# lynet55/robotic-mpc

Hardware: AMD Instinct MI355X
Metric: MPC-steps/sec (whole node), UR10 N=100 dt=0.01 batch; 1/2/4/8 GPU (higher is better)
Workload: dtype f64

## Files before the change

### robotic_mpc_amd/csrc/mpc_core.h

```cpp
#pragma once
#include "mpc_kin.h"
#include "mpc_ipm.h"
#include "mpc_nlp.h"

#define MPC_REP16(X) X(0) X(1) X(2) X(3) X(4) X(5) X(6) X(7) X(8) X(9) X(10) X(11) X(12) X(13) X(14) X(15)
#define MPC_REP4(X) X(0) X(1) X(2) X(3)

namespace mpcb {

constexpr double BOUND_INF = 1e29;

constexpr int L1 = 98;
constexpr int L2N = 62;
constexpr int L2W = 114;

#ifndef MPCB_FUSE
#define MPCB_FUSE 1
#endif
#ifdef MPCB_PROFILE
#define PROF_T0(v) const double v = ex.clock()
#define PROF_ADD(i, v) prof[i] += ex.clock() - v
#else
#define PROF_T0(v)
#define PROF_ADD(i, v)
// ... 590 lines not shown
                            }
                        }
                    });
                }
                ex.par([&](int lane) {
                    ex.put_max(sm.red[0], lane, a_s.at(lane)); ex.put_max(sm.red[1], lane, a_e.at(lane));
                    ex.put_max(sm.red[2], lane, a_i.at(lane)); ex.put_max(sm.red[3], lane, a_c.at(lane));
                });
                rs = fmax(rs, ex.get_max(sm.red[0]));
                re = fmax(re, ex.get_max(sm.red[1]));
                ri = fmax(ri, ex.get_max(sm.red[2]));
                rc = fmax(rc, ex.get_max(sm.red[3]));
            }
            copies([&](int lane, auto nl) {
                constexpr int NL = decltype(nl)::value;
                if (wide) copy_lanes<W2, 0, W2, L2W, false, NL>(v2, ex.smem().w.G2, k0, k1, lane);
                else copy_lanes<W2_LIN, 0, W2, L2N, false, NL>(v2, ex.smem().w.G2, k0, k1, lane);
            });
            PROF_ADD(PF_X3, tn);
        }
        if (res4) { res4[0] = rs; res4[1] = re; res4[2] = ri; res4[3] = rc; }
        PROF_ADD(PF_NLP, t0);
        return cost;
    }

    MPC_PASS void residual_direct(int mode, double a)
    {
        PROF_T0(t0);
        Smem &sm = ex.smem();
        const InstParams &P = sm.P;
        const int Nl = ex.uni(ex.smem().n_hor), NS = Nl + 1;
        double *const G1 = ex.smem().w.G1, *const G2 = ex.smem().w.G2, *const G3 = ex.smem().w.G3;
        double *const Y = ex.pool();
        a = ex.uni(a);
        typename Ex::template PerLane<double> n_g, n_b, n_d, n_m, n_mu, n_c;
        PROF_T0(tx);
        ex.wpar([&](int lane) { n_g.at(lane) = 0; n_b.at(lane) = 0; n_d.at(lane) = 0; n_m.at(lane) = 0; n_mu.at(lane) = 0; n_c.at(lane) = 0; });
        if (mode == 1) {
            constexpr int IPS = 15, R = rounds_for(IPS);
            const int items = NS * IPS;
            for (int base = 0; base < items; base += R * NT) {
                ex.wpar([&](int lane) {
                    D2 cur[R], stp[R];
#pragma unroll
                    for (int r = 0; r < R; r++) {
                        const int e = imin(base + r * NT + lane, items - 1), k = e / IPS, c = 2 * (e - k * IPS);
                        cur[r] = *(MPC_GLOBAL const D2 *)(G1 + (size_t)k * W1 + O_QW + c);
                        stp[r] = *(MPC_GLOBAL const D2 *)(G3 + (size_t)(c >= 18 ? imin(k + 1, Nl) : k) * W3 + O_DW + c);
                    }
#pragma unroll
                    for (int r = 0; r < R; r++) {
                        const int e = base + r * NT + lane;
                        if (e < items) {
                            const int k = e / IPS, c = 2 * (e - k * IPS);
                            const double aa = (c >= 18 && k >= Nl) ? 0.0 : a;
                            D2 v = cur[r];
                            v.x += aa * stp[r].x; v.y += aa * stp[r].y;
                            *(MPC_GLOBAL D2 *)(G1 + (size_t)k * W1 + O_QW + c) = v;
                        }
                    }
                });
            }
        } else {
            ex.wpar([&](int lane) {
                if (lane < NX) gst(G1 + O_QW + 6 + lane, sm.xhat[lane] - gld(G1 + O_X + lane));
                if (lane >= 16 && lane < 16 + NU) gst(G1 + (size_t)Nl * W1 + O_QW + lane - 16, 0.0);
            });
        }
        {
            constexpr int IPS = 24, R = rounds_for(IPS);
            const int items = NS * IPS;
            for (int base = 0; base < items; base += R * NT) {
                ex.wpar([&](int lane) {
                    D2 cur[R], stp[R];
#pragma unroll
                    for (int r = 0; r < R; r++) {
                        const int e = imin(base + r * NT + lane, items - 1), k = e / IPS, q = 2 * (e - k * IPS);
                        cur[r] = *(MPC_GLOBAL const D2 *)(G1 + (size_t)k * W1 + O_QLAM + q);
                        if (mode == 1) stp[r] = *(MPC_GLOBAL const D2 *)(G3 + (size_t)k * W3 + O_DLAM + q);
                    }
                    double ncl = n_c.at(lane);
#pragma unroll
                    for (int r = 0; r < R; r++) {
                        const int e = base + r * NT + lane;
                        if (e < items) {
                            const int k = e / IPS, q = 2 * (e - k * IPS);
                            const bool is_t = q >= 24;
                            const int sc = is_t ? q - 24 : q, j = sc < 12 ? sc : sc - 12;
                            const bool ok = j < 6 ? k < Nl : (k >= 1 && k < Nl);
                            const D2 m = *reinterpret_cast<const D2 *>(&sm.bon[sc]);
                            const bool on0 = ok && m.x != 0.0, on1 = ok && m.y != 0.0;
                            D2 v = cur[r];
                            if (mode == 1) {
                                v.x = ipm::step_floor(on0, v.x, a, stp[r].x); v.y = ipm::step_floor(on1, v.y, a, stp[r].y);
                            } else {
                                v.x = is_t ? ipm::warm_t(on0, v.x) : ipm::warm_lam(on0, v.x);
                                v.y = is_t ? ipm::warm_t(on1, v.y) : ipm::warm_lam(on1, v.y);
                                ncl += (on0 && !is_t ? 1.0 : 0.0) + (on1 && !is_t ? 1.0 : 0.0);
                            }
                            *(MPC_GLOBAL D2 *)(G1 + (size_t)k * W1 + O_QLAM + q) = v;
                        }
                    }
                    n_c.at(lane) = ncl;
                });
            }
        }
        ex.barrier();
        PROF_ADD(PF_X1, tx);
        PROF_T0(ty);
        const int CY = ex.uni(imax(1, imin(ex.smem().pool_n / 6, NS)));
        for (int y0 = 0; y0 < NS; y0 += CY) {
        const int y1 = imin(y0 + CY, NS);
        if (y0 > 0) ex.barrier();
        {
            constexpr int R = rounds_for(NTASK);
            const int items = (imin(y1, Nl) - y0) * NTASK;
            for (int base = 0; base < items; base += R * NT) {
                ex.wpar([&](int lane) {
                    double g[R][12], d[R][12], rr[R];
#pragma unroll
                    for (int r = 0; r < R; r++) {
                        const int e = imax(imin(base + r * NT + lane, items - 1), 0), k = y0 + e / NTASK, i = e - (k - y0) * NTASK;
                        const double *g1 = G1 + (size_t)k * W1 + O_QW, *g2 = G2 + (size_t)k * W2;
                        rr[r] = gld(g2 + O_R + i);
#pragma unroll
                        for (int j = 0; j < 6; j++) { g[r][j] = gld(g2 + O_GQ + i * 6 + j); d[r][j] = gld(g1 + 6 + j); }
                        if (i == 4) {
#pragma unroll
                            for (int j = 0; j < 6; j++) { g[r][6 + j] = gld(g2 + O_GV + j); d[r][6 + j] = gld(g1 + 12 + j); }
                        }
                    }
#pragma unroll
                    for (int r = 0; r < R; r++) {
                        const int e = base + r * NT + lane;
                        if (e < items) {
                            const int k = y0 + e / NTASK, i = e - (k - y0) * NTASK;
                            double v = rr[r];
#pragma unroll
                            for (int j = 0; j < 6; j++) v += g[r][j] * d[r][j];
                            if (i == 4) {
#pragma unroll
                                for (int j = 0; j < 6; j++) v += g[r][6 + j] * d[r][6 + j];
                            }
                            v *= P.w_task[i];
                            Y[(k - y0) * 6 + i] = v;
                            gst(G2 + (size_t)k * W2 + O_Y + i, v);
                        }
                    }
                });
            }
        }
        ex.barrier();
        PROF_ADD(PF_X2, ty);
        PROF_T0(tz);
        {
            constexpr int R = Ex::VGPR_BUDGET <= 256 && rounds_for(6) > 2 ? 2 : rounds_for(6);
            const int items = (y1 - y0) * 6;
            const double dt = P.dt, lm = P.lm;
            auto bounds = [&](int lane, int k, int ci, double val_, double dv, double l_lo, double l_hi, double t_lo, double t_hi,
                              double &rg) {
                const bool hc = ci < 6 ? k < Nl : (k >= 1 && k < Nl);
                const bool blo = hc && sm.bon[ci] != 0.0, bhi = hc && sm.bon[12 + ci] != 0.0;
                const double val = hc ? val_ : 0.0;
                const double ll = blo ? l_lo : 0.0, lu = bhi ? l_hi : 0.0;
                const double itl = fast_rcp(t_lo), itu = fast_rcp(t_hi);
                const double rdl = blo ? dv - (bnd_lo(P, ci) - val) - t_lo : 0.0;
                const double rdu = bhi ? (bnd_hi(P, ci) - val) - dv - t_hi : 0.0;
                const double rml = ll * t_lo, rmu = lu * t_hi;
                double gt = rg;
                rg -= ll; gt -= ll;
                double gam = ll * itl;
                gt += (rml + ll * rdl) * itl;
                rg += lu; gt += lu;
                gam += lu * itu;
                gt -= (rmu + lu * rdu) * itu;
                n_mu.at(lane) += rml + rmu;
                n_d.at(lane) = fmax(n_d.at(lane), fmax(fabs(rdl), fabs(rdu)));
                n_m.at(lane) = fmax(n_m.at(lane), fmax(fabs(rml), fabs(rmu)));
                double *g3 = G3 + (size_t)k * W3, *g2 = G2 + (size_t)k * W2;
                gst(g3 + O_RD + ci, rdl); gst(g3 + O_RD + 12 + ci, rdu);
                gst(g3 + O_RM + ci, rml); gst(g3 + O_RM + 12 + ci, rmu);
                gst(g2 + O_GAM + ci, gam);
                return gt;
            };
            constexpr int RD = 2 * R;
            const int items_d = (y1 - y0) * NX;
            for (int base = 0; base < items; base += R * NT) {
                ex.wpar([&](int lane) {
                    double v[R][12], q[R][13], d[RD][5];
#pragma unroll
                    for (int r = 0; r < R; r++) {
                        const int e = imin(base + r * NT + lane, items - 1), k = y0 + e / 6, j = e - (k - y0) * 6, km = imax(k - 1, 0);
                        const double *g1 = G1 + (size_t)k * W1, *g2 = G2 + (size_t)k * W2, *gm = G1 + (size_t)km * W1;
                        v[r][0] = gld(g1 + O_U + j);      v[r][1] = gld(g1 + O_X + 6 + j);
                        v[r][2] = gld(g1 + O_QW + j);     v[r][3] = gld(g1 + O_QW + 12 + j);
                        v[r][4] = gld(g1 + O_QPI + j);    v[r][5] = gld(g1 + O_QPI + 6 + j);
                        v[r][6] = gld(gm + O_QPI + 6 + j);
                        v[r][7] = gld(g2 + O_GV + j);
                        v[r][8] = gld(g1 + O_QLAM + j);   v[r][9] = gld(g1 + O_QLAM + 12 + j);
                        v[r][10] = gld(g1 + O_QT + j);    v[r][11] = gld(g1 + O_QT + 12 + j);
                        q[r][0] = gld(g1 + O_X + j);  q[r][1] = gld(g1 + O_QW + 6 + j);
#pragma unroll
                        for (int i = 0; i < NTASK; i++) q[r][2 + i] = gld(g2 + O_GQ + i * 6 + j);
                        q[r][7] = v[r][4]; q[r][8] = gld(gm + O_QPI + j);
                        q[r][9] = gld(g1 + O_QLAM + 6 + j);  q[r][10] = gld(g1 + O_QLAM + 18 + j);
                        q[r][11] = gld(g1 + O_QT + 6 + j);   q[r][12] = gld(g1 + O_QT + 18 + j);
                    }
#pragma unroll
                    for (int r = 0; r < RD; r++) {
                        const int e = imin(2 * base + r * NT + lane, items_d - 1), k = y0 + e / NX, i = e - (k - y0) * NX, kn = imin(k + 1, Nl);
                        const double *dw = G1 + (size_t)k * W1 + O_QW;
                        d[r][0] = gld(dw + 6 + i);
                        d[r][1] = gld(dw + (i < 6 ? 12 + i : i - 6));
                        d[r][2] = gld(dw + (i < 6 ? i : i - 6));
                        d[r][3] = gld(G2 + (size_t)k * W2 + O_BD + i);
                        d[r][4] = gld(G1 + (size_t)kn * W1 + O_QW + 6 + i);
                    }
#pragma unroll
                    for (int r = 0; r < R; r++) {
                        const int e = base + r * NT + lane;
                        if (e < items) {
                            const int k = y0 + e / 6, j = e - (k - y0) * 6;
                            const double du = v[r][2], dvv = v[r][3];
                            const double uj = v[r][0] + du, vj = v[r][1] + dvv;
                            const double c2 = P.w_qddot * P.cq[j] * P.cq[j];
                            double *g3 = G3 + (size_t)k * W3, *g2 = G2 + (size_t)k * W2;
                            double rgu = 0.0;
                            if (k < Nl) {
                                rgu = dt * (2.0 * P.w_u * uj + c2 * (uj - vj));
                                rgu += P.b1[j] * v[r][4] + P.b2[j] * v[r][5];
                                rgu += dt * lm * du;
                            }
                            const double gtu = bounds(lane, k, j, v[r][0], du, v[r][8], v[r][9], v[r][10], v[r][11], rgu);
                            gst(g3 + O_RG + j, rgu); gst(g2 + O_GT + j, gtu);
                            double rgv = 0.0;
                            if (k >= 1) {
                                if (k < Nl) {
                                    rgv = dt * (v[r][7] * Y[(k - y0) * 6 + 4] + c2 * (vj - uj));
                                    rgv += P.a12[j] * v[r][4] + P.a22[j] * v[r][5];
                                }
                                rgv += (k < Nl ? dt : 1.0) * lm * dvv;
                                rgv -= v[r][6];
                            }
                            gst(g3 + O_RG + 12 + j, rgv); gst(g2 + O_GT + 12 + j, rgv);
                            const double dq = q[r][1];
                            double rg = 0.0;
                            if (k >= 1) {
                                if (k < Nl) {
                                    double s_ = 0.0;
#pragma unroll
                                    for (int i = 0; i < NTASK; i++) s_ += q[r][2 + i] * Y[(k - y0) * 6 + i];
                                    rg = dt * s_ + q[r][7];
                                }
                                rg += (k < Nl ? dt : 1.0) * lm * dq;
                                rg -= q[r][8];
                            }
                            const double gt = bounds(lane, k, 6 + j, q[r][0], dq, q[r][9], q[r][10], q[r][11], q[r][12], rg);
                            gst(g3 + O_RG + 6 + j, rg); gst(g2 + O_GT + 6 + j, gt);
                            n_g.at(lane) = fmax(n_g.at(lane), fmax(fmax(fabs(rgu), fabs(rgv)), fabs(rg)));
                        }
                    }
#pragma unroll
                    for (int r = 0; r < RD; r++) {
                        const int e = 2 * base + r * NT + lane;
                        if (e < items_d && e < 2 * (base + R * NT)) {
                            const int k = y0 + e / NX, i = e - (k - y0) * NX;
                            double vv = 0.0;
                            if (k < Nl) {
                                if (i < 6) vv = d[r][0] + P.a12[i] * d[r][1] + P.b1[i] * d[r][2];
                                else vv = P.a22[i - 6] * d[r][0] + P.b2[i - 6] * d[r][1];
                                vv += d[r][3] - d[r][4];
                                n_b.at(lane) = fmax(n_b.at(lane), fabs(vv));
                            }
                            gst(G2 + (size_t)k * W2 + O_RB + i, vv);
                        }
                    }
                });
            }
        }
        PROF_ADD(PF_X3, tz);
        }
        ex.par([&](int lane) {
            ex.put_max(sm.red[0], lane, n_g.at(lane)); ex.put_max(sm.red[1], lane, n_b.at(lane));
            ex.put_max(sm.red[2], lane, n_d.at(lane)); ex.put_max(sm.red[3], lane, n_m.at(lane));
            ex.put_sum(sm.red[4], lane, n_mu.at(lane)); ex.put_sum(sm.red[5], lane, n_c.at(lane));
        });
        const double ng = ex.get_max(sm.red[0]), nb = ex.get_max(sm.red[1]), nd = ex.get_max(sm.red[2]), nm = ex.get_max(sm.red[3]);
        const double smu = ex.get_sum(sm.red[4]), nc = ex.get_sum(sm.red[5]);
        ex.par([&](int lane) {
            if ((lane & (WAVE - 1)) == 0) {
                sm.ret[0] = ng; sm.ret[1] = nb; sm.ret[2] = nd; sm.ret[3] = nm; sm.ret[4] = smu;
                if (mode == 0) sm.ret[5] = nc;
            }
        });
        PROF_ADD(PF_RES, t0);
    }

    struct FactLane {
        double b1a, b2a, b1b, b2b, a12a, a22a, a12b, a22b;
        double hu_c;
        double huv_c;
        double lm_c;
        double mqq, mqv, mvq, mvv;
        double qqq, qqv, qvq, qvv;
        int a, b;
        int oqq, oqv, ovv;
    };

    template <int MODE>
    MPC_PASS void fact_pass_t()
    {
        constexpr bool RES = MODE == 1, SEG = MODE == 2;
        PROF_T0(t0);
        Smem &sm = ex.smem();
        const InstParams &P = sm.P;
        const int Nl = ex.uni(ex.smem().n_hor);
        constexpr int WR = 78;
        constexpr int WF = RES ? W4 - O_PM : W4;
        constexpr int FO = RES ? O_PM : 0;
        const ResMap rm = res_map();
        const int CH = RES ? chunk_len_in(rm.scr_n, 2 * (WR + WF), 2 * WR) : chunk_len(2 * (WR + W4), 2 * WR);
        typename Ex::template PerLane<FactLane> fl;
        ex.seq([&](int lane) {
            FactLane &f = fl.at(lane);
            const int a = lane < 36 ? lane / 6 : 0, b = lane < 36 ? lane % 6 : 0;
            f.a = a; f.b = b;
            f.oqq = tri(imin(a, b), imax(a, b)); f.oqv = tri(a, 6 + b); f.ovv = tri(6 + imin(a, b), 6 + imax(a, b));
            f.b1a = P.b1[a]; f.b2a = P.b2[a]; f.b1b = P.b1[b]; f.b2b = P.b2[b];
            f.a12a = P.a12[a]; f.a22a = P.a22[a]; f.a12b = P.a12[b]; f.a22b = P.a22[b];
            const double c2 = P.dt * P.w_qddot * P.cq[a] * P.cq[a];
            f.hu_c = a == b ? P.dt * 2.0 * P.w_u + c2 + P.dt * P.lm : 0.0;
            f.huv_c = a == b ? c2 : 0.0;
            f.lm_c = a == b ? P.dt * P.lm : 0.0;
            f.mqq = f.mqv = f.mvq = f.mvv = 0.0;
            f.qqq = f.qqv = f.qvq = f.qvv = 0.0;
        });
        const double dw0 = P.dt * P.w_task[0], dw1 = P.dt * P.w_task[1], dw2 = P.dt * P.w_task[2], dw3 = P.dt * P.w_task[3],
                     dw4 = P.dt * P.w_task[4];
        auto next_stage = [&](int lane, FactLane &f, double gam_u, int sb) {
            const double fq = f.b1a * f.mqq + f.b2a * f.mvq, fv = f.b1a * f.mqv + f.b2a * f.mvv;
            double r = fq * f.b1b + fv * f.b2b + f.hu_c;
            r += f.a == f.b ? gam_u : 0.0;
            sm.Rt[f.a * 6 + f.b] = r;
            double *St = sm.St2[sb];
            St[f.a * 12 + f.b] = fq;
            St[f.a * 12 + 6 + f.b] = fq * f.a12b + fv * f.a22b - f.huv_c;
            const double cq = f.a12a * f.mqq + f.a22a * f.mvq, cv = f.a12a * f.mqv + f.a22a * f.mvv;
            f.qqq = f.mqq;
            f.qqv = f.mqq * f.a12b + f.mqv * f.a22b;
            f.qvq = cq;
            f.qvv = cq * f.a12b + cv * f.a22b;
            (void)lane;
        };
        int sb = 0;
        const size_t buf = (size_t)(CH + 1) * WR + (size_t)CH * WF;
        auto vr_of = [&](int ci) { return ex.pool() + (size_t)(ci & 1) * buf; };
        auto vf_of = [&](int ci) { return vr_of(ci) + (size_t)(CH + 1) * WR; };
        auto k1_of = [&](int ci) { return Nl - ci * CH; };
        typename Ex::template PerLane<double> pr;
        typename Ex::template PerLane<double> tr, wr;
        typename Ex::template PerLane<D2> ab;
        double b1r[6], b2r[6], a12r[6], a22r[6];
#pragma unroll
        for (int i = 0; i < 6; i++) { b1r[i] = P.b1[i]; b2r[i] = P.b2[i]; a12r[i] = P.a12[i]; a22r[i] = P.a22[i]; }
        typename Ex::template PerLane<double> phi[12];
        int vcur = 0;
        auto vec_sweep = [&](int ci) {
            const int k1c = k1_of(ci), k0c = imax(k1c - CH + 1, 0), klc = imax(k0c - 1, 0);
            const double *vr = vr_of(ci);
            double *vf = vf_of(ci);
            for (int k = k1c; k >= k0c; k--) {
                const double *ric = vr + (size_t)(k - klc) * WR;
                const double *gt = ric + 48, *rbv = ric + 66;
                double *fac = vf + (size_t)(k - k0c) * WF - FO;
                double *kk = RES ? rm.K + (size_t)k * 72 : fac + O_K, *vhp = RES ? rm.VH + (size_t)k * 6 : fac + O_VH;
                double *ep = RES ? rm.E + (size_t)k * 12 : fac + O_E, *pvp = RES ? rm.P + (size_t)k * 12 : fac + O_PV;
                const double *Pn = (k < k1c ? fac + WF : vf_of(ci + 1) - FO) + O_PM;
                const int vnxt = vcur ^ 1;
                ex.await(&sm.prog, Nl - k);
                if (k == Nl) {
                    ex.sub([&](int lane) {
                        if (lane < NX) {
                            const double v = gt[6 + lane];
                            pr.at(lane) = v; ex.share(sm.pv[vcur], lane, v);
                            pvp[lane] = v; fac[O_WV + lane] = 0.0; ep[lane] = 0.0;
                            const int j = lane % 6;
                            D2 c2; c2.x = P.a12[j]; c2.y = P.a22[j];
                            ab.at(lane) = c2;
                        }
                        if (lane < NU) vhp[lane] = 0.0;
                        if (lane == 0) ex.post(&sm.prog1, 0);
                    });
                    continue;
                }
                ex.sub([&](int lane) {
                    double t = 0.0, w = 0.0;
                    if (lane < NX) {
                        double w0 = 0.0, w1 = 0.0;
#pragma unroll
                        for (int j = 0; j < NX; j += 2) { w0 += Pn[tri_sym(lane, j)] * rbv[j]; w1 += Pn[tri_sym(lane, j + 1)] * rbv[j + 1]; }
                        w = w0 + w1;
                        t = pr.at(lane) + w;
                    }
                    tr.at(lane) = t; wr.at(lane) = w;
                    ex.share(sm.mt2[vcur], lane < NX ? lane : NX, t);
                });
                ex.sub([&](int lane) {
                    const double t = tr.at(lane), w = wr.at(lane);
                    double tv[12];
#pragma unroll
                    for (int i = 0; i < NX; i++) tv[i] = ex.gather(sm.mt2[vcur], i, t);
                    const double oq = ex.shr6(sm.mt2[vcur], lane, t);
                    if (lane < NX) {
                        const int j = lane;
                        double hu[6];
#pragma unroll
                        for (int m = 0; m < 6; m++) hu[m] = gt[m] + b1r[m] * tv[m] + b2r[m] * tv[6 + m];
                        const D2 c2 = ab.at(lane);
                        double pj = gt[6 + j] + (j < 6 ? t : c2.x * oq + c2.y * t);
                        double s0 = 0.0, s1 = 0.0;
#pragma unroll
                        for (int m = 0; m < 6; m += 2) { s0 += kk[m * 12 + j] * hu[m]; s1 += kk[(m + 1) * 12 + j] * hu[m + 1]; }
                        pj -= s0 + s1;
                        pr.at(lane) = pj; ex.share(sm.pv[vnxt], lane, pj);
                        pvp[j] = pj;
                        fac[O_WV + j] = w;
                        const int i6 = j < 6 ? j : j - 6;
                        double v0 = 0.0, v1 = 0.0;
#pragma unroll
                        for (int m = 0; m < 6; m += 2) { v0 += fac[O_RI + i6 * 6 + m] * hu[m]; v1 += fac[O_RI + i6 * 6 + m + 1] * hu[m + 1]; }
                        const double vh = v0 + v1;
                        if (j < 6) vhp[j] = vh;
                        ep[j] = rbv[j] - (j < 6 ? P.b1[i6] : P.b2[i6]) * vh;
                    }
                    if (lane == 0) ex.post(&sm.prog1, Nl - k);
                });
                vcur = vnxt;
            }
        };
        constexpr int NBW = Ex::BG_WAVES;
        ex.par([&](int lane) {
            if (lane == 0) { ex.post(&sm.prog, -1); ex.post(&sm.prog1, -1); ex.post(&sm.flg[0], NBW); ex.post(&sm.flg[1], 0); }
        });
        load_rect<WR, O_GQ, W2>(vr_of(0), ex.smem().w.G2, imax(imax(Nl - CH + 1, 0) - 1, 0), Nl);
        const int nwin = (Nl + CH) / CH;
        PROF_T0(ts);
        ex.pipeline3(nwin, [&](int ci) {
            const int k1 = k1_of(ci), k0 = imax(k1 - CH + 1, 0), kl = imax(k0 - 1, 0);
            double *vr = vr_of(ci), *vf = vf_of(ci);
            ex.await(&sm.flg[0], NBW * (ci + 1));
            if (ci >= 2) ex.await(&sm.flg[1], NBW * ci);
            for (int k = k1; k >= k0; k--) {
                const double *ric = vr + (size_t)(k - kl) * WR;
                const double *ricd = ric - WR;
                double *fac = vf + (size_t)(k - k0) * WF - FO;
                double *kk = RES ? rm.K + (size_t)k * 72 : fac + O_K;
                const double *gam = ric + 36;
                if (k == Nl) {
                    ex.seq([&](int lane) {
                        const double lmN = ex.smem().P.lm;
                        for (int e = lane; e < NPM; e += WAVE) {
                            double v = 0.0;
#pragma unroll
                            for (int i = 0; i < NX; i++) v = e == tri(i, i) ? lmN : v;
                            fac[O_PM + e] = v;
                        }
                        if (lane < 36) {
                            FactLane &f = fl.at(lane);
                            f.mqv = f.mvq = 0.0;
                            f.mqq = f.mvv = f.a == f.b ? lmN : 0.0;
                            next_stage(lane, f, ricd[36 + f.a], sb);
                        }
                        if (lane == 0) ex.post(&sm.prog, 0);
                    });
                    continue;
                }
#ifndef MPCB_DIAG_NO_B
                ex.seq([&](int lane) {
                    const double *St = sm.St2[sb];
                    double A_[6][6];
#pragma unroll
                    for (int i = 0; i < 6; i++)
#pragma unroll
                        for (int j = 0; j <= i; j++) A_[i][j] = sm.Rt[i * 6 + j];
                    double dinv[6];
#pragma unroll
                    for (int j = 0; j < 6; j++) {
#ifdef MPCB_DIAG_NO_LDL
                        dinv[j] = A_[j][j]; continue;
#endif
                        dinv[j] = fast_rcp(A_[j][j]);
                        double lj[6];
#pragma unroll
                        for (int i = j + 1; i < 6; i++) lj[i] = A_[i][j] * dinv[j];
#pragma unroll
                        for (int i = j + 1; i < 6; i++)
#pragma unroll
                            for (int r = j + 1; r <= i; r++) A_[i][r] -= lj[i] * A_[r][j];
#pragma unroll
                        for (int i = j + 1; i < 6; i++) A_[i][j] = lj[i];
                    }
                    if (lane < 18) {
                        double x[6];
                        const int col = lane < 12 ? lane : 0;
#pragma unroll
                        for (int i = 0; i < 6; i++) x[i] = St[i * 12 + col];
#pragma unroll
                        for (int i = 0; i < 6; i++) x[i] = lane < 12 ? x[i] : (i == lane - 12 ? 1.0 : 0.0);
#pragma unroll
                        for (int j = 0; j < 6; j++) {
#pragma unroll
                            for (int i = j + 1; i < 6; i++) x[i] -= A_[i][j] * x[j];
                        }
#pragma unroll
                        for (int i = 0; i < 6; i++) x[i] *= dinv[i];
#pragma unroll
                        for (int j = 5; j >= 0; j--) {
#pragma unroll
                            for (int i = 0; i < j; i++) x[i] -= A_[j][i] * x[j];
                        }
                        if (lane < 12) {
#pragma unroll
                            for (int i = 0; i < 6; i++) kk[i * 12 + lane] = x[i];
                        } else {
#pragma unroll
                            for (int i = 0; i < 6; i++) fac[O_RI + i * 6 + (lane - 12)] = x[i];
                        }
                    }
                });
#endif
                ex.seq([&](int lane) {
#ifdef MPCB_DIAG_NO_CA
                    if (lane == 0) ex.post(&sm.prog, Nl - k);
                    return;
#endif
                    if (lane < 36) {
                        FactLane &f = fl.at(lane);
                        if (k > 0) {
                            const double *St = sm.St2[sb];
                            const double *gq = ric, *gv = ric + 30;
                            const double ga0 = gq[f.a], ga1 = gq[6 + f.a], ga2 = gq[12 + f.a], ga3 = gq[18 + f.a], ga4 = gq[24 + f.a];
                            const double gb0 = gq[f.b], gb1 = gq[6 + f.b], gb2 = gq[12 + f.b], gb3 = gq[18 + f.b], gb4 = gq[24 + f.b];
                            const double gva = gv[f.a], gvb = gv[f.b];
                            const double gam_q = gam[6 + f.a], gam_u = ricd[36 + f.a];
                            double sa[6], sva[6], kb[6], kvb[6];
#pragma unroll
                            for (int m = 0; m < 6; m++) { sa[m] = St[m * 12 + f.a]; sva[m] = St[m * 12 + 6 + f.a]; }
#pragma unroll
                            for (int m = 0; m < 6; m++) { kb[m] = kk[m * 12 + f.b]; kvb[m] = kk[m * 12 + 6 + f.b]; }
#if defined(__HIP_DEVICE_COMPILE__)
                            asm volatile("" ::: "memory");
#endif
                            double pqq = f.qqq + (dw0 * ga0 * gb0 + dw1 * ga1 * gb1 + dw2 * ga2 * gb2 + dw3 * ga3 * gb3 + dw4 * ga4 * gb4) + f.lm_c;
                            double pqv = f.qqv + dw4 * ga4 * gvb;
                            double pvq = f.qvq + dw4 * gva * gb4;
                            double pvv = f.qvv + dw4 * gva * gvb + (f.huv_c + f.lm_c);
                            pqq += f.a == f.b ? gam_q : 0.0;
#pragma unroll
                            for (int m = 0; m < 6; m++) {
                                pqq -= sa[m] * kb[m]; pqv -= sa[m] * kvb[m];
                                pvq -= sva[m] * kb[m]; pvv -= sva[m] * kvb[m];
                            }
                            f.mqq = pqq; f.mqv = pqv; f.mvq = pvq; f.mvv = pvv;
                            next_stage(lane, f, gam_u, sb ^ 1);
                            if (f.a <= f.b) { fac[O_PM + f.oqq] = pqq; fac[O_PM + f.ovv] = pvv; }
                            fac[O_PM + f.oqv] = pqv;
                        }
                    }
                    if (lane == 0) ex.post(&sm.prog, Nl - k);
                });
                sb ^= 1;
            }
            }, [&](int ci) {
#ifndef MPCB_DIAG_NO_VEC
                vec_sweep(ci);
#endif
            }, [&](int ci, int lane, auto nl) {
                constexpr int NL = decltype(nl)::value;
                const int k1 = k1_of(ci), k0 = imax(k1 - CH + 1, 0);
                const int nk1 = k0 - 1, nk0 = imax(nk1 - CH + 1, 0), nkl = imax(nk0 - 1, 0);
                const int pk1 = k1 + CH, pk0 = k1 + 1;
                if (ci > 0) ex.await(&sm.prog1, Nl - pk0);
                if (nk1 >= 0) copy_lanes<WR, O_GQ, W2, WR, true, NL>(vr_of(ci + 1), ex.smem().w.G2, nkl, nk1, lane);
                if ((lane & (WAVE - 1)) == 0) ex.post_add(&sm.flg[0], 1);
                if (ci > 0) copy_lanes<WF, FO, W4, WF, false, NL>(vf_of(ci - 1), ex.smem().w.G4, pk0, pk1, lane);
                ex.await(&sm.prog1, Nl - k1);
                if ((lane & (WAVE - 1)) == 0) ex.post_add(&sm.flg[1], 1);
                if constexpr (RES || SEG) {
#ifndef MPCB_DIAG_NO_PHI
                    if (lane < WAVE) {
                        const int L = SEG ? (reg_ok() ? RL : seg_map().L) : rm.L;
                        for (int k = imin(k1, Nl - 1); k >= k0; k--) {
                            ex.await(&sm.prog, Nl - k);
                            const double *kk = RES ? rm.K + (size_t)k * 72 : vf_of(ci) + (size_t)(k - k0) * WF - FO + O_K;
                            const int c = k / L;
                            const bool first = ex.uni(k == imin((c + 1) * L, Nl) - 1), last = ex.uni(k == c * L);
                            const D2 kv2 = reinterpret_cast<const D2 *>(kk)[(lane & (WAVE - 1)) < 36 ? (lane & (WAVE - 1)) : 0];
                            auto Kat = [&](int idx) { return ex.lane_value(kk, idx, (idx & 1) ? kv2.y : kv2.x, idx >> 1); };
                            {
                                double ph[12], g[6], nw[12];
#pragma unroll
                                for (int j = 0; j < 12; j++) ph[j] = first ? (j == lane ? 1.0 : 0.0) : phi[j].at(lane);
#pragma unroll
                                for (int m = 0; m < 6; m++) g[m] = ph[m] * b1r[m] + ph[6 + m] * b2r[m];
#pragma unroll
                                for (int j = 0; j < 6; j++) {
                                    double s0 = ph[j], s1 = a12r[j] * ph[j] + a22r[j] * ph[6 + j];
#pragma unroll
                                    for (int m = 0; m < 6; m++) { s0 -= g[m] * Kat(m * 12 + j); s1 -= g[m] * Kat(m * 12 + 6 + j); }
                                    nw[j] = s0; nw[6 + j] = s1;
                                }
#pragma unroll
                                for (int j = 0; j < 12; j++) phi[j].at(lane) = nw[j];
                                if (last && lane < NX) {
                                    if (SEG) {
#pragma unroll
                                        for (int j = 0; j < 12; j++) gst(ex.smem().w.PH + (size_t)c * 144 + lane * 12 + j, nw[j]);
                                    } else {
#pragma unroll
                                        for (int j = 0; j < 12; j++) rm.PHI[(size_t)c * 144 + lane * 12 + j] = nw[j];
                                    }
                                }
                            }
                        }
                    }
#endif
                }
            });
        PROF_ADD(PF_SEQ_FACT, ts);
        {
            const int k1 = k1_of(nwin - 1);
            copy_rect<WF, FO, W4, WF, false>(vf_of(nwin - 1), ex.smem().w.G4, 0, k1);
        }
        PROF_ADD(PF_FACT, t0);
    }

    MPC_PASS void corrector_bwd_pass(double sigma_mu)
    {
        PROF_T0(t0);
        Smem &sm = ex.smem();
        const InstParams &P = sm.P;
        const int Nl = ex.uni(ex.smem().n_hor);
        constexpr int WLT = 50;
        constexpr int L3 = 90;
        constexpr int C_DLAM = 42, C_DT = 66;
        constexpr int WGR = 30;
        constexpr int WK = 72, WW = 50;
        constexpr int WC = 12;
        constexpr int WRM = 24, WHP = 30;
        constexpr int C_PV = 18;
        constexpr int PER = WLT + L3 + WGR + WK + WW + WC + WRM + WHP;
        const int CH = chunk_len(2 * PER, 0);
        typename Ex::template PerLane<D2> ab;
        typename Ex::template PerLane<double> pr;
        double b1r[6], b2r[6];
#pragma unroll
        for (int i = 0; i < 6; i++) { b1r[i] = P.b1[i]; b2r[i] = P.b2[i]; }
        ex.seq([&](int lane) {
            const int j = lane % 6;
            D2 v; v.x = P.a12[j]; v.y = P.a22[j];
            ab.at(lane) = v;
            pr.at(lane) = 0.0;
        });
        auto carve = [&](int sel, double *&vlt, double *&v3, double *&vgr, double *&vk, double *&vw, double *&vc, double *&orm,
                         double *&ohp) {
            vlt = ex.pool() + (size_t)sel * CH * PER;
            v3 = vlt + (size_t)CH * WLT; vgr = v3 + (size_t)CH * L3; vk = vgr + (size_t)CH * WGR;
            vw = vk + (size_t)CH * WK; vc = vw + (size_t)CH * WW; orm = vc + (size_t)CH * WC; ohp = orm + (size_t)CH * WRM;
        };
        int cur = 0, bsel = 0;
        {
            double *vlt, *v3, *vgr, *vk, *vw, *vc, *orm, *ohp;
            carve(0, vlt, v3, vgr, vk, vw, vc, orm, ohp);
            const int f0 = imax(Nl - CH + 1, 0);
            copies([&](int lane, auto nl) {
                constexpr int NL = decltype(nl)::value;
                copy_lanes<48, O_QLAM, W1, WLT, true, NL>(vlt, ex.smem().w.G1, f0, Nl, lane);
                copy_lanes<42, 0, W3, L3, true, NL>(v3, ex.smem().w.G3, f0, Nl, lane);
                copy_lanes<48, O_DLAM, W3, L3, true, NL>(v3 + C_DLAM, ex.smem().w.G3, f0, Nl, lane);
                copy_lanes<WGR, O_GT, W2, WGR, true, NL>(vgr, ex.smem().w.G2, f0, Nl, lane);
                copy_lanes<WK, O_K, W4, WK, true, NL>(vk, ex.smem().w.G4, f0, Nl, lane);
                copy_lanes<48, O_WV, W4, WW, true, NL>(vw, ex.smem().w.G4, f0, Nl, lane);
            });
        }
        for (int k1 = Nl; k1 >= 0; k1 -= CH, bsel ^= 1) {
            const int k0 = imax(k1 - CH + 1, 0);
            double *vlt, *v3, *vgr, *vk, *vw, *vc, *orm, *ohp;
            carve(bsel, vlt, v3, vgr, vk, vw, vc, orm, ohp);
            double *nlt, *n3, *ngr, *nk, *nw, *nc_, *prm, *php;
            carve(bsel ^ 1, nlt, n3, ngr, nk, nw, nc_, prm, php);
            const int nk1 = k0 - 1, nk0 = imax(nk1 - CH + 1, 0);
            ex.par([&](int lane) {
                const int rows = k1 - k0 + 1;
                for (int e = lane; e < rows * NB; e += NT) {
                    const int s = e / NB, j = e - s * NB, k = k0 + s;
                    const double *lt = vlt + (size_t)s * WLT;
                    const double *r3 = v3 + (size_t)s * L3;
                    double *rmo = orm + (size_t)s * WRM;
                    const bool hc = has_comp(Nl, k, j);
                    const bool blo = hc && bnd_lo(P, j) > -BOUND_INF, bhi = hc && bnd_hi(P, j) < BOUND_INF;
                    const double ll = lt[j], tl = lt[24 + j], lu = lt[12 + j], tu = lt[36 + j];
                    const double dll = r3[C_DLAM + j], dtl = r3[C_DT + j], dlu = r3[C_DLAM + 12 + j], dtu = r3[C_DT + 12 + j];
                    const double rdl = r3[18 + j], rdu = r3[18 + 12 + j];
                    double gt = r3[j];
                    double rml, rmu;
                    gt += ipm::corrector_side(blo, ll, tl, dll, dtl, rdl, sigma_mu, rml);
                    gt -= ipm::corrector_side(bhi, lu, tu, dlu, dtu, rdu, sigma_mu, rmu);
                    if (hc) vgr[(size_t)s * WGR + j] = gt;
                    rmo[j] = rml; rmo[12 + j] = rmu;
                }
            });
            ex.par([&](int lane) {
                const int rows = k1 - k0 + 1;
                for (int e = lane; e < rows * NX; e += NT) {
                    const int s = e / NX, j = e - s * NX, k = k0 + s;
                    const double *gt = vgr + (size_t)s * WGR, *w = vw + (size_t)s * WW, *kf = vk + (size_t)s * WK;
                    double v = 0.0;
                    if (k < Nl) {
                        v = gt[6 + j] + (j < 6 ? w[j] : P.a12[j - 6] * w[j - 6] + P.a22[j - 6] * w[j]);
#pragma unroll
                        for (int m = 0; m < 6; m++) v -= kf[m * 12 + j] * (gt[m] + P.b1[m] * w[m] + P.b2[m] * w[6 + m]);
                    }
                    vc[(size_t)s * WC + j] = v;
                }
            });
            PROF_T0(ts);
            ex.overlap([&]() {
            for (int k = k1; k >= k0; k--) {
                const double *gt = vgr + (size_t)(k - k0) * WGR;
                const double *cv = vc + (size_t)(k - k0) * WC;
                const double *kf = vk + (size_t)(k - k0) * WK;
                double *hp = ohp + (size_t)(k - k0) * WHP;
                const int nxt = cur ^ 1;
                if (k == Nl) {
                    ex.seq([&](int lane) {
                        if (lane < NX) {
                            const double v = gt[6 + lane];
                            pr.at(lane) = v; ex.share(sm.pv[cur], lane, v);
                            hp[C_PV + lane] = v;
                            hp[6 + lane] = 0.0;
                        }
                        if (lane < NU) hp[lane] = 0.0;
                    });
                    continue;
                }
                ex.seq([&](int lane) {
                    const int jc = lane < NX ? lane : 0;
                    double kc[6];
#pragma unroll
                    for (int i = 0; i < 6; i++) kc[i] = kf[i * 12 + jc];
                    const double ck = cv[jc];
                    const double mine = pr.at(lane);
                    double pn[12];
#pragma unroll
                    for (int i = 0; i < NX; i++) pn[i] = ex.gather(sm.pv[cur], i, mine);
                    const double oq = ex.shr6(sm.pv[cur], lane, mine);
                    double acc0 = 0.0, acc1 = 0.0;
#pragma unroll
                    for (int i = 0; i < 6; i += 2) {
                        acc0 += kc[i] * (b1r[i] * pn[i] + b2r[i] * pn[6 + i]);
                        acc1 += kc[i + 1] * (b1r[i + 1] * pn[i + 1] + b2r[i + 1] * pn[7 + i]);
                    }
                    const D2 c2 = ab.at(lane);
                    const double at = lane < 6 ? mine : c2.x * oq + c2.y * mine;
                    const double pj = ck + (at - (acc0 + acc1));
                    pr.at(lane) = pj;
                    if (lane < NX) {
                        ex.share(sm.pv[nxt], lane, pj);
                        hp[C_PV + lane] = pj;
                    }
                });
                cur = nxt;
            }
            }, [&](int lane, auto nl) {
                constexpr int NL = decltype(nl)::value;
                if (nk1 >= 0) {
                    copy_lanes<48, O_QLAM, W1, WLT, true, NL>(nlt, ex.smem().w.G1, nk0, nk1, lane);
                    copy_lanes<42, 0, W3, L3, true, NL>(n3, ex.smem().w.G3, nk0, nk1, lane);
                    copy_lanes<48, O_DLAM, W3, L3, true, NL>(n3 + C_DLAM, ex.smem().w.G3, nk0, nk1, lane);
                    copy_lanes<WGR, O_GT, W2, WGR, true, NL>(ngr, ex.smem().w.G2, nk0, nk1, lane);
                    copy_lanes<WK, O_K, W4, WK, true, NL>(nk, ex.smem().w.G4, nk0, nk1, lane);
                    copy_lanes<48, O_WV, W4, WW, true, NL>(nw, ex.smem().w.G4, nk0, nk1, lane);
                }
                if (k1 < Nl) {
                    copy_lanes<WRM, O_RM, W3, WRM, false, NL>(prm, ex.smem().w.G3, k1 + 1, k1 + CH, lane);
                    copy_lanes<WHP, O_VH, W4, WHP, false, NL>(php, ex.smem().w.G4, k1 + 1, k1 + CH, lane);
                }
            });
            PROF_ADD(PF_SEQ_BWD, ts);
            ex.par([&](int lane) {
                const int rows = k1 - k0 + 1;
                for (int e = lane; e < rows * NX; e += NT) {
                    const int s = e / NX, j = e - s * NX, k = k0 + s;
                    if (k >= Nl) continue;
                    const double *gt = vgr + (size_t)s * WGR, *w = vw + (size_t)s * WW, *ri = w + 12;
                    const double *pn = (s + 1 < rows ? ohp + (size_t)(s + 1) * WHP : php) + C_PV;
                    const int i6 = j < 6 ? j : j - 6;
                    double v0 = 0.0, v1 = 0.0;
#pragma unroll
                    for (int m = 0; m < 6; m += 2) {
                        const double h0 = gt[m] + P.b1[m] * (pn[m] + w[m]) + P.b2[m] * (pn[6 + m] + w[6 + m]);
                        const double h1 = gt[m + 1] + P.b1[m + 1] * (pn[m + 1] + w[m + 1]) + P.b2[m + 1] * (pn[7 + m] + w[7 + m]);
                        v0 += ri[i6 * 6 + m] * h0; v1 += ri[i6 * 6 + m + 1] * h1;
                    }
                    const double vh = v0 + v1;
                    double *hp = ohp + (size_t)s * WHP;
                    if (j < 6) hp[j] = vh;
                    hp[6 + j] = gt[18 + j] - (j < 6 ? P.b1[i6] : P.b2[i6]) * vh;
                }
            });
            if (k0 == 0) {
                copies([&](int lane, auto nl) {
                    constexpr int NL = decltype(nl)::value;
                    copy_lanes<WRM, O_RM, W3, WRM, false, NL>(orm, ex.smem().w.G3, k0, k1, lane);
                    copy_lanes<WHP, O_VH, W4, WHP, false, NL>(ohp, ex.smem().w.G4, k0, k1, lane);
                });
            }
        }
        PROF_ADD(PF_BWD, t0);
    }

    template <bool AFFINE, bool FAST = false>
    MPC_PASS double forward_step_pass()
    {
        static_assert(!FAST || !AFFINE, "the fast path takes the full step");
        PROF_T0(t0);
        Smem &sm = ex.smem();
        const InstParams &P = sm.P;
        const int Nl = ex.uni(ex.smem().n_hor);
        constexpr int WLT = 50, WR = 50, WO = 78;
        constexpr int LF = AFFINE ? W4_AFF : W4_FWD;
        constexpr int PER = LF + WLT + WR + WO;
#ifndef MPCB_FWD_BLK
#define MPCB_FWD_BLK 4
#endif
        constexpr int BLK = MPCB_FWD_BLK;
        const int CH = chunk_len(2 * PER, 0);
        const int NCH = (Nl + CH) / CH;
        double *const pool = ex.pool();
        typename Ex::template PerLane<D2> ab, bb;
        typename Ex::template PerLane<double> dxr;
        typename Ex::template PerLane<double> r_al, r_a0, r_a1, r_a2;
        ex.par([&](int lane) {
            const int j = (lane & (WAVE - 1)) % 6;
            D2 v; v.x = P.a12[j]; v.y = P.a22[j];
            ab.at(lane) = v;
            D2 u; u.x = P.b1[j]; u.y = P.b2[j];
            bb.at(lane) = u;
            dxr.at(lane) = 0.0;
            if (lane < NX) ex.share(sm.dx[0], lane, 0.0);
            r_al.at(lane) = 1.0; r_a0.at(lane) = 0.0; r_a1.at(lane) = 0.0; r_a2.at(lane) = 0.0;
            if (lane == 0) ex.post(&sm.prog, -1);
        });
        int cur = 0;
        {
            double *q4 = pool, *qlt = q4 + (size_t)CH * LF, *qr = qlt + (size_t)CH * WLT;
            const int e1 = imin(CH - 1, Nl);
            copies([&](int lane, auto nl) {
                constexpr int NL = decltype(nl)::value;
                copy_lanes<LF, 0, W4, LF, true, NL>(q4, ex.smem().w.G4, 0, e1, lane);
                if (FAST) copy_lanes<18, 0, W1, WLT, true, NL>(qlt, ex.smem().w.G1, 0, e1, lane);
                else {
                copy_lanes<48, O_QLAM, W1, WLT, true, NL>(qlt, ex.smem().w.G1, 0, e1, lane);
                copy_lanes<48, O_RD, W3, WR, true, NL>(qr, ex.smem().w.G3, 0, e1, lane);
                }
            });
        }
        for (int ci = 0; ci < NCH; ci++) {
            const int k0 = ci * CH, k1 = imin(k0 + CH - 1, Nl);
            double *v4 = pool + (size_t)(ci & 1) * CH * PER;
            double *vlt = v4 + (size_t)CH * LF;
            double *vr = vlt + (size_t)CH * WLT;
            double *vo = vr + (size_t)CH * WR;
            double *n4 = pool + (size_t)((ci + 1) & 1) * CH * PER, *nlt = n4 + (size_t)CH * LF,
                   *nr = nlt + (size_t)CH * WLT, *po = nr + (size_t)CH * WR;
            const int nk0 = k1 + 1, nk1 = imin(nk0 + CH - 1, Nl);
            PROF_T0(ts);
            ex.overlap3([&]() {
            for (int k = k0; k <= k1; k++) {
                const int nxt = cur ^ 1;
                const double *fac = v4 + (size_t)(k - k0) * LF;
                double *o = vo + (size_t)(k - k0) * WO;
                ex.seq([&](int lane) {
                    const int lc = lane < NX ? lane : 0, i = lc < 6 ? lc : lc - 6;
                    double kr[12];
#pragma unroll
                    for (int j = 0; j < NX; j++) kr[j] = fac[O_K + i * 12 + j];
                    const double ek = fac[O_E + lc];
                    const double own = dxr.at(lane);
                    double dxv[12];
#pragma unroll
                    for (int j = 0; j < NX; j++) dxv[j] = ex.gather(sm.dx[cur], j, own);
                    const double ov = ex.shl6(sm.dx[cur], lane, own);
                    double s0 = 0.0, s1 = 0.0;
#pragma unroll
                    for (int j = 0; j < NX; j += 2) {
// ... 1305 lines not shown
```

### robotic_mpc_amd/csrc/mpc_layout.h

```cpp
#pragma once

#include <stddef.h>

#define MPC_HD __host__ __device__ __forceinline__
#define MPC_PASS __host__ __device__ __noinline__

namespace mpcb {

constexpr int WAVE = 64;
constexpr int NWV_MAX = 8;
constexpr int NT_MAX = WAVE * NWV_MAX;
constexpr int NQ = 6;
constexpr int NX = 12;
constexpr int NU = 6;
constexpr int NW = 18;
constexpr int NB = 12;
constexpr int NL = 24;
constexpr int NTASK = 5;

constexpr int W1 = 96;
constexpr int O_X = 0, O_U = 12, O_QW = 18, O_QPI = 36, O_QLAM = 48, O_QT = 72;
constexpr int W2 = 112;
constexpr int O_R = 0;
constexpr int O_Y = 5;
constexpr int O_BD = 12;
constexpr int O_GQ = 24;
constexpr int O_GV = 54;
constexpr int O_GAM = 60;
constexpr int O_GT = 72;
constexpr int O_RB = 90;
constexpr int W2_LIN = 60;
constexpr int W3 = 144;
constexpr int O_RG = 0, O_RD = 18, O_RM = 42;
constexpr int O_DW = 66;
constexpr int O_DPI = 84;
constexpr int O_DLAM = 96, O_DT = 120;
constexpr int W4 = 228;
constexpr int O_K = 0;
constexpr int O_VH = 72;
constexpr int O_E = 78;
constexpr int O_PV = 90;
constexpr int O_PM = 102;
constexpr int NPM = 78;
constexpr int O_WV = 180;
constexpr int O_RI = 192;
constexpr int W4_AFF = O_PV;
constexpr int W4_FWD = O_WV;
constexpr int W5 = 116;
constexpr int O_NPI = 0, O_NLAM = 12, O_NT = 36, O_TX = 60, O_TU = 72, O_MW = 78;

constexpr int STAGE_DOUBLES = W1 + W2 + W3 + W4 + W5;
constexpr int ST_Z = 0;
constexpr int ST_LIN_COST = 12;
constexpr int ST_X0_MW = 13;
constexpr int ST_LIN_VALID = 25;
constexpr int ST_FAST = 26;
constexpr int ST_CUR = 28;
constexpr int ST_PROF = 32;
constexpr int NPROF = 16;
constexpr int STATE_DOUBLES = 64;

struct Robot {
    double place[7][12];
    double axis[6][3];
    double t_ee[3];
};

struct InstParams {
    double dt, tol, qp_tol, w_u, w_qddot, px_ref, vy_ref, integ;
    double wcv[6], q0[6], qdot0[6], qmin[6], qmax[6], umin[6], umax[6];
    double coeffs[6];
    double w_task[5];
    double lm;
    double a12[6], a22[6], b1[6], b2[6];
    double cq[6];
    double tol_eq, tol_ineq, tol_comp;
    double n_hor;
    double fast_off;
};

struct Problem {
    int batch;
    int N;
    int Nsim;
    int solver_type;
    int max_iter;
    int qp_iter_max;
    int fixed_step;
    int precision;
};

struct Outputs {
    double *z;
    double *u;
    double *ee_pose;
    double *ee_rpy;
    double *ee_vel;
    int *status;
    int *sqp_iter;
    int *qp_iter;
    double *residuals;
    double *cost;
    double *solver_time;
    double *errors;
    double *plant_time;
};

struct StepIO {
    const double *xhat;
    double *u0;
    int *status;
    int *sqp_iter;
    int *qp_iter;
    double *residuals;
    double *cost;
    double *solver_time;
    double *x_pred;
    double *u_pred;
    const double *yref = nullptr;
    int ref_changed = 0;
};

struct TaskRef {
    const double *y;
};

struct Ws {
    double *G1, *G2, *G3, *G4, *G5, *PH, *state;
};
constexpr int SEG_L_FULL = 7, SEG_J_FULL = 16, SEG_L_HALF = 5, SEG_J_HALF = 8, SEG_POOL_FULL = 17000;
MPC_HD size_t ws_phi_doubles(int N) { return (size_t)((N + SEG_L_HALF - 1) / SEG_L_HALF + 1) * 144; }
constexpr int RS_PER_STAGE_L = 72 + 6 + 12 + 12;
MPC_HD bool lay_resident_ok(int N, int pool_n, int groups)
{
    const int NS = N + 1, scr = pool_n - (NS * RS_PER_STAGE_L + groups * 144);
    return scr >= 4096 && scr >= NS * 30 + 2 * groups * 12 + 16;
}
MPC_HD bool lay_segment_ok(int N, int pool_n, int groups)
{
    if (groups < 8 || pool_n < SEG_POOL_FULL || lay_resident_ok(N, pool_n, groups)) return false;
    const int Jc = groups < SEG_J_FULL ? groups : SEG_J_FULL, T = SEG_L_FULL * Jc;
    const int scr = pool_n - ((T + 1) * RS_PER_STAGE_L + Jc * 144);
    return scr >= (T + 1) * 30 + 2 * groups * 12 + 64;
}

MPC_HD int tri(int r, int c) { return r * 12 - (r * (r - 1)) / 2 + (c - r); }
MPC_HD int tri_sym(int i, int j) { return i <= j ? tri(i, j) : tri(j, i); }

MPC_HD size_t ws_doubles_per_instance(int N) { return (size_t)(N + 1) * STAGE_DOUBLES + ws_phi_doubles(N) + STATE_DOUBLES; }

MPC_HD Ws ws_carve(double *base, int N)
{
    const size_t n1 = (size_t)N + 1;
    Ws w;
    double *p = base;
    w.G1 = p; p += n1 * W1;
    w.G2 = p; p += n1 * W2;
    w.G3 = p; p += n1 * W3;
    w.G4 = p; p += n1 * W4;
    w.G5 = p; p += n1 * W5;
    w.PH = p; p += ws_phi_doubles(N);
    w.state = p;
    return w;
}

constexpr int LOG_ROWS = 46, LOGB = 8;

struct Smem {
    InstParams P;
    alignas(16) Robot rb;
    Ws w;
    int n_hor, pool_n;
    int prog;
    int prog1;
    int flg[2];
    int flg_pad;
    alignas(16) double mt2[2][16];
    alignas(16) double pv[2][12];
    alignas(16) double Rt[36];
    alignas(16) double St2[2][72];
    alignas(16) double Kf[72];
    alignas(16) double dx[2][12];
    alignas(16) double ret[8];
    alignas(16) double cen[4];
    alignas(16) double bon[24];
    alignas(16) double red[8][NWV_MAX];
    alignas(16) double xhat[12];
    alignas(16) double u0[6];
    alignas(16) double logv[48];
    alignas(16) double logbuf[LOG_ROWS][LOGB];
};

constexpr int POOL_MIN_DOUBLES = 2048;
constexpr int POOL_DEFAULT_DOUBLES = 19456;
constexpr int LDS_CU_BYTES = 160 * 1024;
MPC_HD int lay_pool_doubles(int sims_per_cu)
{
    const int fixed = (int)sizeof(Smem) + 64;
    int bytes = LDS_CU_BYTES / (sims_per_cu < 1 ? 1 : sims_per_cu) - fixed;
    if (bytes > POOL_DEFAULT_DOUBLES * 8) bytes = POOL_DEFAULT_DOUBLES * 8;
    if (bytes < POOL_MIN_DOUBLES * 8) bytes = POOL_MIN_DOUBLES * 8;
    return (bytes / 16) * 2;
}

}
```

Measured before the change: 1.565 million.

## Move gain solve off the Riccati critical path into the vector-sweep waves

The Riccati recursion no longer runs a separate LDL solve for the gains K and R^-1 on the critical path. Each of the 36 lanes now folds the LDL elimination directly into its own Schur-complement update, using double-buffered Rt2/St2 tiles. The raw R, S entries are stored, and the vector-sweep waves later factor them to produce K and R^-1 columns. A new progress flag (prog2) lets consumers wait until those gains are ready. This shortens the serial chain per stage, at the cost of redundant per-lane factorization and extra synchronization.

Result: slower. 1.389 million (-11.2%).

```diff
diff --git a/robotic_mpc_amd/csrc/mpc_core.h b/robotic_mpc_amd/csrc/mpc_core.h
--- a/robotic_mpc_amd/csrc/mpc_core.h
+++ b/robotic_mpc_amd/csrc/mpc_core.h
@@ -916,6 +916,7 @@
         double huv_c;
         double lm_c;
         double mqq, mqv, mvq, mvv;
+        double r, s0, s1;
         double qqq, qqv, qvq, qvv;
         int a, b;
         int oqq, oqv, ovv;
@@ -947,6 +948,7 @@
             f.huv_c = a == b ? c2 : 0.0;
             f.lm_c = a == b ? P.dt * P.lm : 0.0;
             f.mqq = f.mqv = f.mvq = f.mvv = 0.0;
+            f.r = f.s0 = f.s1 = 0.0;
             f.qqq = f.qqv = f.qvq = f.qvv = 0.0;
         });
         const double dw0 = P.dt * P.w_task[0], dw1 = P.dt * P.w_task[1], dw2 = P.dt * P.w_task[2], dw3 = P.dt * P.w_task[3],
@@ -955,10 +957,12 @@
             const double fq = f.b1a * f.mqq + f.b2a * f.mvq, fv = f.b1a * f.mqv + f.b2a * f.mvv;
             double r = fq * f.b1b + fv * f.b2b + f.hu_c;
             r += f.a == f.b ? gam_u : 0.0;
-            sm.Rt[f.a * 6 + f.b] = r;
+            sm.Rt2[sb][f.a * 6 + f.b] = r;
             double *St = sm.St2[sb];
+            const double sv = fq * f.a12b + fv * f.a22b - f.huv_c;
             St[f.a * 12 + f.b] = fq;
-            St[f.a * 12 + 6 + f.b] = fq * f.a12b + fv * f.a22b - f.huv_c;
+            St[f.a * 12 + 6 + f.b] = sv;
+            f.r = r; f.s0 = fq; f.s1 = sv;
             const double cq = f.a12a * f.mqq + f.a22a * f.mvq, cv = f.a12a * f.mqv + f.a22a * f.mvv;
             f.qqq = f.mqq;
             f.qqv = f.mqq * f.a12b + f.mqv * f.a22b;
@@ -973,6 +977,8 @@
         auto k1_of = [&](int ci) { return Nl - ci * CH; };
         typename Ex::template PerLane<double> pr;
         typename Ex::template PerLane<double> tr, wr;
+        struct GainCol { double k[6], ri[6]; };
+        typename Ex::template PerLane<GainCol> gc;
         typename Ex::template PerLane<D2> ab;
         double b1r[6], b2r[6], a12r[6], a22r[6];
 #pragma unroll
@@ -1003,19 +1009,53 @@
                             ab.at(lane) = c2;
                         }
                         if (lane < NU) vhp[lane] = 0.0;
-                        if (lane == 0) ex.post(&sm.prog1, 0);
+                        if (lane == 0) { ex.post(&sm.prog2, 0); ex.post(&sm.prog1, 0); }
                     });
                     continue;
                 }
                 ex.sub([&](int lane) {
                     double t = 0.0, w = 0.0;
                     if (lane < NX) {
+                        const int i6 = lane < 6 ? lane : lane - 6;
+                        double A_[6][6];
+#pragma unroll
+                        for (int i = 0; i < 6; i++)
+#pragma unroll
+                            for (int j = 0; j <= i; j++) A_[i][j] = fac[O_RI + i * 6 + j];
+                        double x[6], z[6];
+#pragma unroll
+                        for (int i = 0; i < 6; i++) { x[i] = kk[i * 12 + lane]; z[i] = i == i6 ? 1.0 : 0.0; }
                         double w0 = 0.0, w1 = 0.0;
 #pragma unroll
                         for (int j = 0; j < NX; j += 2) { w0 += Pn[tri_sym(lane, j)] * rbv[j]; w1 += Pn[tri_sym(lane, j + 1)] * rbv[j + 1]; }
                         w = w0 + w1;
                         t = pr.at(lane) + w;
-                    }
+                        double dinv[6];
+#pragma unroll
+                        for (int j = 0; j < 6; j++) {
+                            dinv[j] = fast_rcp(A_[j][j]);
+                            double lj[6];
+#pragma unroll
+                            for (int i = j + 1; i < 6; i++) lj[i] = A_[i][j] * dinv[j];
+#pragma unroll
+                            for (int i = j + 1; i < 6; i++)
+#pragma unroll
+                                for (int r = j + 1; r <= i; r++) A_[i][r] -= lj[i] * A_[r][j];
+#pragma unroll
+                            for (int i = j + 1; i < 6; i++) { A_[i][j] = lj[i]; x[i] -= lj[i] * x[j]; z[i] -= lj[i] * z[j]; }
+                        }
+#pragma unroll
+                        for (int i = 0; i < 6; i++) { x[i] *= dinv[i]; z[i] *= dinv[i]; }
+#pragma unroll
+                        for (int j = 5; j >= 0; j--) {
+#pragma unroll
+                            for (int i = 0; i < j; i++) { x[i] -= A_[j][i] * x[j]; z[i] -= A_[j][i] * z[j]; }
+                        }
+                        GainCol &g = gc.at(lane);
+#pragma unroll
+                        for (int i = 0; i < 6; i++) { kk[i * 12 + lane] = x[i]; g.k[i] = x[i]; g.ri[i] = z[i]; }
+                    }
+                    if (lane == 0) ex.post(&sm.prog2, Nl - k);
                     tr.at(lane) = t; wr.at(lane) = w;
                     ex.share(sm.mt2[vcur], lane < NX ? lane : NX, t);
                 });
@@ -1033,8 +1073,9 @@
                         const D2 c2 = ab.at(lane);
                         double pj = gt[6 + j] + (j < 6 ? t : c2.x * oq + c2.y * t);
                         double s0 = 0.0, s1 = 0.0;
-#pragma unroll
-                        for (int m = 0; m < 6; m += 2) { s0 += kk[m * 12 + j] * hu[m]; s1 += kk[(m + 1) * 12 + j] * hu[m + 1]; }
+                        const GainCol &g = gc.at(lane);
+#pragma unroll
+                        for (int m = 0; m < 6; m += 2) { s0 += g.k[m] * hu[m]; s1 += g.k[m + 1] * hu[m + 1]; }
                         pj -= s0 + s1;
                         pr.at(lane) = pj; ex.share(sm.pv[vnxt], lane, pj);
                         pvp[j] = pj;
@@ -1042,9 +1083,13 @@
                         const int i6 = j < 6 ? j : j - 6;
                         double v0 = 0.0, v1 = 0.0;
 #pragma unroll
-                        for (int m = 0; m < 6; m += 2) { v0 += fac[O_RI + i6 * 6 + m] * hu[m]; v1 += fac[O_RI + i6 * 6 + m + 1] * hu[m + 1]; }
+                        for (int m = 0; m < 6; m += 2) { v0 += g.ri[m] * hu[m]; v1 += g.ri[m + 1] * hu[m + 1]; }
                         const double vh = v0 + v1;
-                        if (j < 6) vhp[j] = vh;
+                        if (j < 6) {
+                            vhp[j] = vh;
+#pragma unroll
+                            for (int m = 0; m < 6; m++) fac[O_RI + m * 6 + j] = g.ri[m];
+                        }
                         ep[j] = rbv[j] - (j < 6 ? P.b1[i6] : P.b2[i6]) * vh;
                     }
                     if (lane == 0) ex.post(&sm.prog1, Nl - k);
@@ -1054,7 +1099,7 @@
         };
         constexpr int NBW = Ex::BG_WAVES;
         ex.par([&](int lane) {
-            if (lane == 0) { ex.post(&sm.prog, -1); ex.post(&sm.prog1, -1); ex.post(&sm.flg[0], NBW); ex.post(&sm.flg[1], 0); }
+            if (lane == 0) { ex.post(&sm.prog, -1); ex.post(&sm.prog1, -1); ex.post(&sm.prog2, -1); ex.post(&sm.flg[0], NBW); ex.post(&sm.flg[1], 0); }
         });
         load_rect<WR, O_GQ, W2>(vr_of(0), ex.smem().w.G2, imax(imax(Nl - CH + 1, 0) - 1, 0), Nl);
         const int nwin = (Nl + CH) / CH;
@@ -1089,79 +1134,28 @@
                     });
                     continue;
                 }
-#ifndef MPCB_DIAG_NO_B
                 ex.seq([&](int lane) {
-                    const double *St = sm.St2[sb];
-                    double A_[6][6];
-#pragma unroll
-                    for (int i = 0; i < 6; i++)
-#pragma unroll
-                        for (int j = 0; j <= i; j++) A_[i][j] = sm.Rt[i * 6 + j];
-                    double dinv[6];
-#pragma unroll
-                    for (int j = 0; j < 6; j++) {
-#ifdef MPCB_DIAG_NO_LDL
-                        dinv[j] = A_[j][j]; continue;
-#endif
-                        dinv[j] = fast_rcp(A_[j][j]);
-                        double lj[6];
-#pragma unroll
-                        for (int i = j + 1; i < 6; i++) lj[i] = A_[i][j] * dinv[j];
-#pragma unroll
-                        for (int i = j + 1; i < 6; i++)
-#pragma unroll
-                            for (int r = j + 1; r <= i; r++) A_[i][r] -= lj[i] * A_[r][j];
-#pragma unroll
-                        for (int i = j + 1; i < 6; i++) A_[i][j] = lj[i];
-                    }
-                    if (lane < 18) {
-                        double x[6];
-                        const int col = lane < 12 ? lane : 0;
-#pragma unroll
-                        for (int i = 0; i < 6; i++) x[i] = St[i * 12 + col];
-#pragma unroll
-                        for (int i = 0; i < 6; i++) x[i] = lane < 12 ? x[i] : (i == lane - 12 ? 1.0 : 0.0);
-#pragma unroll
-                        for (int j = 0; j < 6; j++) {
-#pragma unroll
-                            for (int i = j + 1; i < 6; i++) x[i] -= A_[i][j] * x[j];
-                        }
-#pragma unroll
-                        for (int i = 0; i < 6; i++) x[i] *= dinv[i];
-#pragma unroll
-                        for (int j = 5; j >= 0; j--) {
-#pragma unroll
-                            for (int i = 0; i < j; i++) x[i] -= A_[j][i] * x[j];
-                        }
-                        if (lane < 12) {
-#pragma unroll
-                            for (int i = 0; i < 6; i++) kk[i * 12 + lane] = x[i];
-                        } else {
-#pragma unroll
-                            for (int i = 0; i < 6; i++) fac[O_RI + i * 6 + (lane - 12)] = x[i];
-                        }
-                    }
-                });
-#endif
-                ex.seq([&](int lane) {
-#ifdef MPCB_DIAG_NO_CA
-                    if (lane == 0) ex.post(&sm.prog, Nl - k);
-                    return;
-#endif
                     if (lane < 36) {
                         FactLane &f = fl.at(lane);
                         if (k > 0) {
                             const double *St = sm.St2[sb];
                             const double *gq = ric, *gv = ric + 30;
+                            double A_[6][6];
+#pragma unroll
+                            for (int i = 0; i < 6; i++)
+#pragma unroll
+                                for (int j = 0; j <= i; j++) A_[i][j] = sm.Rt2[sb][i * 6 + j];
+                            double ya[6], yva[6], yb[6], yvb[6];
+#pragma unroll
+                            for (int m = 0; m < 6; m++) { ya[m] = St[m * 12 + f.a]; yva[m] = St[m * 12 + 6 + f.a]; }
+#pragma unroll
+                            for (int m = 0; m < 6; m++) { yb[m] = St[m * 12 + f.b]; yvb[m] = St[m * 12 + 6 + f.b]; }
                             const double ga0 = gq[f.a], ga1 = gq[6 + f.a], ga2 = gq[12 + f.a], ga3 = gq[18 + f.a], ga4 = gq[24 + f.a];
                             const double gb0 = gq[f.b], gb1 = gq[6 + f.b], gb2 = gq[12 + f.b], gb3 = gq[18 + f.b], gb4 = gq[24 + f.b];
                             const double gva = gv[f.a], gvb = gv[f.b];
                             const double gam_q = gam[6 + f.a], gam_u = ricd[36 + f.a];
-                            double sa[6], sva[6], kb[6], kvb[6];
-#pragma unroll
-                            for (int m = 0; m < 6; m++) { sa[m] = St[m * 12 + f.a]; sva[m] = St[m * 12 + 6 + f.a]; }
-#pragma unroll
-                            for (int m = 0; m < 6; m++) { kb[m] = kk[m * 12 + f.b]; kvb[m] = kk[m * 12 + 6 + f.b]; }
+                            fac[O_RI + f.a * 6 + f.b] = f.r;
+                            kk[f.a * 12 + f.b] = f.s0; kk[f.a * 12 + 6 + f.b] = f.s1;
 #if defined(__HIP_DEVICE_COMPILE__)
                             asm volatile("" ::: "memory");
 #endif
@@ -1171,14 +1165,31 @@
                             double pvv = f.qvv + dw4 * gva * gvb + (f.huv_c + f.lm_c);
                             pqq += f.a == f.b ? gam_q : 0.0;
 #pragma unroll
-                            for (int m = 0; m < 6; m++) {
-                                pqq -= sa[m] * kb[m]; pqv -= sa[m] * kvb[m];
-                                pvq -= sva[m] * kb[m]; pvv -= sva[m] * kvb[m];
+                            for (int j = 0; j < 6; j++) {
+                                const double dj = fast_rcp(A_[j][j]);
+                                double lj[6];
+#pragma unroll
+                                for (int i = j + 1; i < 6; i++) lj[i] = A_[i][j] * dj;
+#pragma unroll
+                                for (int i = j + 1; i < 6; i++)
+#pragma unroll
+                                    for (int r = j + 1; r <= i; r++) A_[i][r] -= lj[i] * A_[r][j];
+#pragma unroll
+                                for (int i = j + 1; i < 6; i++) {
+                                    ya[i] -= lj[i] * ya[j]; yva[i] -= lj[i] * yva[j];
+                                    yb[i] -= lj[i] * yb[j]; yvb[i] -= lj[i] * yvb[j];
+                                }
+                                const double za = ya[j] * dj, zva = yva[j] * dj;
+                                pqq -= za * yb[j]; pqv -= za * yvb[j];
+                                pvq -= zva * yb[j]; pvv -= zva * yvb[j];
                             }
                             f.mqq = pqq; f.mqv = pqv; f.mvq = pvq; f.mvv = pvv;
                             next_stage(lane, f, gam_u, sb ^ 1);
                             if (f.a <= f.b) { fac[O_PM + f.oqq] = pqq; fac[O_PM + f.ovv] = pvv; }
                             fac[O_PM + f.oqv] = pqv;
+                        } else {
+                            fac[O_RI + f.a * 6 + f.b] = f.r;
+                            kk[f.a * 12 + f.b] = f.s0; kk[f.a * 12 + 6 + f.b] = f.s1;
                         }
                     }
                     if (lane == 0) ex.post(&sm.prog, Nl - k);
@@ -1186,9 +1197,7 @@
                 sb ^= 1;
             }
             }, [&](int ci) {
-#ifndef MPCB_DIAG_NO_VEC
                 vec_sweep(ci);
-#endif
             }, [&](int ci, int lane, auto nl) {
                 constexpr int NL = decltype(nl)::value;
                 const int k1 = k1_of(ci), k0 = imax(k1 - CH + 1, 0);
@@ -1205,7 +1214,7 @@
                     if (lane < WAVE) {
                         const int L = SEG ? (reg_ok() ? RL : seg_map().L) : rm.L;
                         for (int k = imin(k1, Nl - 1); k >= k0; k--) {
-                            ex.await(&sm.prog, Nl - k);
+                            ex.await(&sm.prog2, Nl - k);
                             const double *kk = RES ? rm.K + (size_t)k * 72 : vf_of(ci) + (size_t)(k - k0) * WF - FO + O_K;
                             const int c = k / L;
                             const bool first = ex.uni(k == imin((c + 1) * L, Nl) - 1), last = ex.uni(k == c * L);
diff --git a/robotic_mpc_amd/csrc/mpc_layout.h b/robotic_mpc_amd/csrc/mpc_layout.h
--- a/robotic_mpc_amd/csrc/mpc_layout.h
+++ b/robotic_mpc_amd/csrc/mpc_layout.h
@@ -174,12 +174,12 @@
     int prog;
     int prog1;
     int flg[2];
-    int flg_pad;
+    int prog2;
     alignas(16) double mt2[2][16];
     alignas(16) double pv[2][12];
-    alignas(16) double Rt[36];
+    alignas(16) double Rt2[2][36];
     alignas(16) double St2[2][72];
-    alignas(16) double Kf[72];
+    alignas(16) double spare[36];
     alignas(16) double dx[2][12];
     alignas(16) double ret[8];
     alignas(16) double cen[4];
```
